# haoyuhsu/autovfx

Measured on AMD Instinct MI355X. Metric: rendered frames/sec at 1920x1080, 3M Gaussians, higher is better.
Workload: dtype f32; 1 GPU; C3: 3M synthetic Gaussians, 1920x1080, 800-frame orbit (BASELINE configs[2], per-GPU shard); P=3000000, sh_coeffs=16, width=1920, height=1080, tiles=8160, boundary=GaussianRasterizer.forward + RGBA8 pack per frame, parallelism=frame-parallel x1, streams_per_gpu=11, stream_driver=pipelined, n_ranks_seen=1

## Files before the change

autovfx_amd/csrc/gsr_binning.hip:

```cpp
#include "gsr_device.h"

#ifdef GSR_KERNEL_TRACE
__device__ unsigned long long* g_binning_trace = nullptr;
extern "C" __attribute__((visibility("default"))) int gsr_debug_set_binning_trace(void* device_words) {
    return (int)hipMemcpyToSymbol(HIP_SYMBOL(g_binning_trace), &device_words, sizeof device_words);
}
#define GSR_BTRACE(id, slot) do { if (threadIdx.x == 0 && g_binning_trace) g_binning_trace[(size_t)(id) * 8 + (slot)] = wall_clock64(); } while (0)
#else
#define GSR_BTRACE(id, slot) do { } while (0)
#endif

namespace gsr {
namespace {

constexpr int kPairTile = kExpandTile;
constexpr int kPairsPerLane = kPairTile / 256;
constexpr int kMaxDoneWords = 4096;
static_assert(kDupTile == 1024, "256 lanes x 4 consecutive positions");

__device__ __forceinline__ uint32_t block_sum_256(uint32_t v, uint32_t* scratch) {
#pragma unroll
    for (int d = 32; d >= 1; d >>= 1) v += (uint32_t)__shfl_xor((int)v, d);
    if ((threadIdx.x & 63) == 0) scratch[threadIdx.x >> 6] = v;
    __syncthreads();
    const uint32_t total = scratch[0] + scratch[1] + scratch[2] + scratch[3];
    __syncthreads();
    return total;
}

__device__ __forceinline__ uint32_t block_exclusive_256(uint32_t mine, uint32_t* s_wave, uint32_t* total) {
    const int lane = threadIdx.x & 63, wave = threadIdx.x >> 6;
    uint32_t incl = mine;
#pragma unroll
    for (int d = 1; d < 64; d <<= 1) {
        const uint32_t o = (uint32_t)__shfl_up((int)incl, d);
        if (lane >= d) incl += o;
    }
    if (lane == 63) s_wave[wave] = incl;
    __syncthreads();
    uint32_t before = incl - mine, all = 0;
#pragma unroll
    for (int w = 0; w < 4; ++w) {
        if (w < wave) before += s_wave[w];
        all += s_wave[w];
    }
    __syncthreads();
    *total = all;
    return before;
}

__device__ __forceinline__ bool rec_is_masked(uint32_t wh) { return (wh & 0xFFFFu) * (wh >> 16) <= kMaskTiles; }

__device__ __forceinline__ unsigned long long done_bits(const uint32_t* rows, int row_words, uint32_t ty, uint32_t x0, uint32_t w) {
    const uint32_t* r = rows + ty * (uint32_t)row_words;
    const uint32_t wi = x0 >> 5, sh = x0 & 31u;
    const uint32_t last = (uint32_t)row_words - 1u;
    const unsigned long long a = (unsigned long long)r[min(wi, last)] | ((unsigned long long)(wi + 1 <= last ? r[wi + 1] : 0u) << 32);
    unsigned long long v = a >> sh;
    if (sh + w > 64u) v |= (unsigned long long)(wi + 2 <= last ? r[wi + 2] : 0u) << (64u - sh);
    return w >= 64u ? v : v & ((1ull << w) - 1ull);
}

__device__ __forceinline__ unsigned long long done_rect(const uint32_t* rows, int row_words, uint32_t xy0, uint32_t wh) {
    const uint32_t x0 = xy0 & 0xFFFFu, y0 = xy0 >> 16, w = wh & 0xFFFFu, h = wh >> 16;
    unsigned long long d = 0ull;
    for (uint32_t j = 0; j < h; ++j) d |= done_bits(rows, row_words, y0 + j, x0, w) << (j * w);
    return d;
}

struct TileWalker {
    uint32_t x0, y0, width;
    bool masked;
    unsigned long long mask;
    float inv_width;
    const uint32_t* runs;
    const uint32_t* incl;
    const uint32_t* done;
    int row_words;
    uint32_t height, row, ca, cb, col_base, cur;

    __device__ __forceinline__ void load_run() {
        if (runs != nullptr) {
            const uint32_t r = runs[row];
            ca = r & 0xFFFFu; cb = r >> 16;
        } else {
            ca = x0; cb = x0 + width;
        }
    }
    __device__ __forceinline__ void load_word() {
        const uint32_t lo = max(ca, col_base), hi = min(cb, col_base + 32u);
// ... 84 lines not shown
    __shared__ float4 s_reg1[4][64];
    __shared__ uint4 s_geo[4][64];
    __shared__ uint32_t s_rows[4][64];
    __shared__ uint32_t s_live[4][64];
    const int tid = threadIdx.x, lane = tid & 63;
    const int V = a.V;
    const int k0 = (int)blockIdx.x * kDupTile + 4 * tid;
    GSR_BTRACE(blockIdx.x, 0);
    uint32_t gid[4] = {0u, 0u, 0u, 0u};
    if (k0 + 3 < V) {
        const uint4 g = *reinterpret_cast<const uint4*>(a.depth_order + k0);
        gid[0] = g.x; gid[1] = g.y; gid[2] = g.z; gid[3] = g.w;
    } else {
#pragma unroll
        for (int j = 0; j < 4; ++j)
            if (k0 + j < V) gid[j] = a.depth_order[k0 + j];
    }
    uint4 rec[4];
    uint32_t count[4];
    bool any_rows = false;
#pragma unroll
    for (int j = 0; j < 4; ++j) {
        rec[j] = make_uint4(0u, 0u, 0u, 0u);
        count[j] = 0u;
        if (k0 + j < V) {
            rec[j] = *reinterpret_cast<const uint4*>(a.bins + gid[j]);
            if (rec_is_masked(rec[j].y)) count[j] = (uint32_t)__popc(rec[j].z) + (uint32_t)__popc(rec[j].w);
            else if (a.tile_cull) {
                any_rows = true;
                rec[j].z += a.pool_first[gid[j] >> 8] + a.pool_group_first[gid[j] >> a.pool_group_shift];
            }
        }
    }
    const unsigned long long any_big = __ballot(any_rows);
    GSR_BTRACE(blockIdx.x, 1);
    if (any_big != 0ull) {
        const int wave = tid >> 6;
#pragma unroll
        for (int j = 0; j < 4; ++j) {
            const bool large = k0 + j < V && !rec_is_masked(rec[j].y);
            const uint32_t h = large ? rec[j].y >> 16 : 0u;
            const uint32_t pool_at = rec[j].z;
            bool walk = false;
            if (large) {
                if (pool_at > a.pool_rows || h > a.pool_rows - pool_at) {
                    rec[j].z = 0xFFFFFFFFu;
                    count[j] = (rec[j].y & 0xFFFFu) * h;
                    rec[j].w = count[j];
                } else {
                    walk = true;
                }
            }
            const uint32_t rows = walk ? h : 0u;
            uint32_t rincl = rows;
#pragma unroll
            for (int d = 1; d < 64; d <<= 1) {
                const uint32_t o = (uint32_t)__shfl_up((int)rincl, d);
                if (lane >= d) rincl += o;
            }
            const uint32_t total = (uint32_t)__shfl((int)rincl, 63);
            if (total != 0u) {
                if (walk) {
                    const float4* rr = reinterpret_cast<const float4*>(a.raster + gid[j]);
                    const float4 r0 = rr[0], r1 = rr[1];
                    const LiveRegion g = live_region(r0.z, r0.w, r1.x, r1.w);
                    s_reg0[wave][lane] = make_float4(g.A, g.B, g.C, g.beta);
                    s_reg1[wave][lane] = make_float4(g.u_ext, g.v_ext, r0.x, r0.y);
                    s_geo[wave][lane] = make_uint4(rec[j].x, (rec[j].y & 0xFFFFu) | ((uint32_t)g.kind << 16), pool_at, 0u);
                }
                s_rows[wave][lane] = rincl;
                s_live[wave][lane] = 0u;
                GSR_WAIT_LDS();
                __builtin_amdgcn_wave_barrier();
                for (uint32_t t0 = 0; t0 < total; t0 += 64u) {
                    const uint32_t t = t0 + (uint32_t)lane;
                    int lo = 64;
                    uint32_t len = 0u, before = 0u, pool_row = 0u, run = 0u;
                    if (t < total) {
                        lo = 0;
                        int hi = 63;
#pragma unroll
                        for (int step = 0; step < 6; ++step) {
                            const int mid = (lo + hi) >> 1;
                            if (s_rows[wave][mid] > t) hi = mid; else lo = mid + 1;
                        }
                        const uint32_t r = t - (lo > 0 ? s_rows[wave][lo - 1] : 0u);
                        const float4 q0 = s_reg0[wave][lo], q1 = s_reg1[wave][lo];
                        const uint4 ge = s_geo[wave][lo];
                        LiveRegion g;
                        g.A = q0.x; g.B = q0.y; g.C = q0.z; g.beta = q0.w; g.u_ext = q1.x; g.v_ext = q1.y; g.kind = (int)(ge.y >> 16);
                        const uint32_t x0 = ge.x & 0xFFFFu, y0 = ge.x >> 16, w = ge.y & 0xFFFFu;
                        int ca, cb;
                        row_run(g, q1.z, q1.w, (int)(y0 + r), (int)x0, (int)(x0 + w), &ca, &cb);
                        run = (uint32_t)ca | ((uint32_t)cb << 16);
                        len = (uint32_t)(cb - ca);
                        pool_row = ge.z + r;
                        before = s_live[wave][lo];
                    }
                    uint32_t incl_len = len;
#pragma unroll
                    for (int d = 1; d < 64; d <<= 1) {
                        const uint32_t o_len = (uint32_t)__shfl_up((int)incl_len, d);
                        const int o_seg = __shfl_up(lo, d);
                        if (lane >= d && o_seg == lo) incl_len += o_len;
                    }
                    GSR_WAIT_LDS();
                    __builtin_amdgcn_wave_barrier();
                    if (t < total) {
                        a.run_pool[pool_row] = run;
                        a.run_incl[pool_row] = before + incl_len;
                        if (len != 0u) atomicAdd(&s_live[wave][lo], len);
                    }
                    GSR_WAIT_LDS();
// ... 94 lines not shown
            slabs[0].pairs = mine[(below - 1u) & 3u];
            if (slabs_host != nullptr) slabs_host[0].pairs = mine[(below - 1u) & 3u];
        }
    }
}

__device__ __forceinline__ void load_done_rows(uint32_t* s_done, const uint32_t* __restrict__ done_rows, int words) {
    for (int i = threadIdx.x; i < words; i += 256) s_done[i] = done_rows[i];
    __syncthreads();
}

__global__ void __launch_bounds__(256, 7) slab_recount_kernel(BinningArrays a, int slab) {
    extern __shared__ uint32_t s_done[];
    __shared__ uint32_t s_wave[4];
    __shared__ uint4 s_geo[4][64];
    __shared__ uint32_t s_rows[4][64];
    __shared__ uint32_t s_live[4][64];
    GSR_BTRACE(8192 + blockIdx.x, 0);
    const SlabInfo info = a.slabs[slab];
    const uint32_t first = info.first, end = min(info.end, (uint32_t)a.V);
    const uint32_t k0 = first + blockIdx.x * (uint32_t)kDupTile + 4u * threadIdx.x;
    if (first + blockIdx.x * (uint32_t)kDupTile >= end) return;
    GSR_BTRACE(8192 + blockIdx.x, 1);
    load_done_rows(s_done, a.done_rows, a.grid_y * a.row_words);
    uint32_t done_tiles = 0;
    for (int i = threadIdx.x; i < a.grid_y * a.row_words; i += 256) {
        const int word = i % a.row_words;
        const uint32_t cols = (uint32_t)min(32, a.grid_x - 32 * word);
        done_tiles += (uint32_t)__popc(s_done[i] & (cols >= 32u ? ~0u : (1u << cols) - 1u));
    }
    const bool nothing_left = block_sum_256(done_tiles, s_wave) == (uint32_t)(a.grid_x * a.grid_y);
    GSR_BTRACE(8192 + blockIdx.x, 2);
    uint32_t count[4];
    uint4 rec[4];
#pragma unroll
    for (int j = 0; j < 4; ++j) {
        count[j] = 0u;
        rec[j] = make_uint4(0u, 0u, 0u, 0u);
        const uint32_t k = k0 + j;
        if (k >= end || nothing_left) continue;
        rec[j] = a.sorted_bins[k];
        if (rec[j].y == 0u || !rec_is_masked(rec[j].y)) continue;
        const unsigned long long m = (unsigned long long)rec[j].z | ((unsigned long long)rec[j].w << 32);
        const unsigned long long left = m & ~done_rect(s_done, a.row_words, rec[j].x, rec[j].y);
        count[j] = (uint32_t)__popcll(left);
    }
    GSR_BTRACE(8192 + blockIdx.x, 3);
    {
        const int lane = threadIdx.x & 63, wave = threadIdx.x >> 6;
#pragma unroll
        for (int j = 0; j < 4; ++j) {
            const bool large = k0 + j < end && rec[j].y != 0u && !rec_is_masked(rec[j].y);
            const uint32_t rows = large ? rec[j].y >> 16 : 0u;
            uint32_t rincl = rows;
#pragma unroll
            for (int d = 1; d < 64; d <<= 1) {
                const uint32_t o = (uint32_t)__shfl_up((int)rincl, d);
                if (lane >= d) rincl += o;
            }
            const uint32_t total = (uint32_t)__shfl((int)rincl, 63);
            if (total == 0u) continue;
            s_geo[wave][lane] = rec[j];
            s_rows[wave][lane] = rincl;
            s_live[wave][lane] = 0u;
            GSR_WAIT_LDS();
            __builtin_amdgcn_wave_barrier();
            for (uint32_t t0 = 0; t0 < total; t0 += 64u) {
                const uint32_t t = t0 + (uint32_t)lane;
                if (t < total) {
                    int lo = 0, hi = 63;
#pragma unroll
                    for (int step = 0; step < 6; ++step) {
                        const int mid = (lo + hi) >> 1;
                        if (s_rows[wave][mid] > t) hi = mid; else lo = mid + 1;
                    }
                    const uint32_t r = t - (lo > 0 ? s_rows[wave][lo - 1] : 0u);
                    const uint4 ge = s_geo[wave][lo];
                    const uint32_t x0 = ge.x & 0xFFFFu, y0 = ge.x >> 16, w = ge.y & 0xFFFFu;
                    uint32_t ca = x0, cb = x0 + w;
                    if (ge.z != 0xFFFFFFFFu) {
                        const uint32_t run = a.run_pool[ge.z + r];
                        ca = run & 0xFFFFu; cb = run >> 16;
                    }
                    uint32_t n = 0u;
                    for (uint32_t col = ca & ~31u; col < cb; col += 32u) {
                        const uint32_t lo_c = max(ca, col), hi_c = min(cb, col + 32u);
                        const uint32_t len = hi_c - lo_c;
                        uint32_t bits = (len >= 32u ? ~0u : ((1u << len) - 1u)) << (lo_c - col);
                        bits &= ~s_done[(y0 + r) * (uint32_t)a.row_words + (col >> 5)];
                        n += (uint32_t)__popc(bits);
                    }
                    if (n != 0u) atomicAdd(&s_live[wave][lo], n);
                }
            }
            GSR_WAIT_LDS();
            __builtin_amdgcn_wave_barrier();
            if (large) count[j] = s_live[wave][lane];
            __builtin_amdgcn_wave_barrier();
        }
    }
    GSR_BTRACE(8192 + blockIdx.x, 4);
    const uint32_t mine = count[0] + count[1] + count[2] + count[3];
    uint32_t tile_total;
    const uint32_t before = block_exclusive_256(mine, s_wave, &tile_total);
    const uint32_t emitting = (count[0] != 0u) + (count[1] != 0u) + (count[2] != 0u) + (count[3] != 0u);
    const uint32_t tile_emitting = block_sum_256(emitting, s_wave);
    if (threadIdx.x == 0) {
        a.slab_tile_totals[blockIdx.x] = tile_total;
        a.slab_tile_totals[a.tiles_p + blockIdx.x] = tile_emitting;
    }
    uint32_t run = before;
#pragma unroll
    for (int j = 0; j < 4; ++j) {
// ... 2 lines not shown
    }
    GSR_BTRACE(8192 + blockIdx.x, 5);
}

__global__ void __launch_bounds__(256) slab_compact_kernel(BinningArrays a, int slab) {
    __shared__ uint32_t s_scratch[4];
    __shared__ uint32_t s_wave[4];
    const SlabInfo info = a.slabs[slab];
    const uint32_t first = info.first, end = min(info.end, (uint32_t)a.V);
    const uint32_t tiles = end > first ? (end - first + kDupTile - 1) / kDupTile : 0u;
    const uint32_t* __restrict__ pair_totals = a.slab_tile_totals;
    const uint32_t* __restrict__ emit_totals = a.slab_tile_totals + a.tiles_p;
    if (blockIdx.x == 0) {
        uint32_t pp = 0, ee = 0;
        for (uint32_t t = threadIdx.x; t < tiles; t += 256) { pp += pair_totals[t]; ee += emit_totals[t]; }
        const uint32_t all_pairs = block_sum_256(pp, s_scratch);
        const uint32_t all_emit = block_sum_256(ee, s_scratch);
        if (threadIdx.x == 0) {
            a.slabs[slab].pairs = all_pairs; a.slabs[slab].emitters = all_emit;
            if (a.slabs_host != nullptr) a.slabs_host[slab].pairs = all_pairs;
        }
    }
    if (blockIdx.x >= tiles) return;
    uint32_t pp = 0, ee = 0;
    for (uint32_t t = threadIdx.x; t < blockIdx.x; t += 256) { pp += pair_totals[t]; ee += emit_totals[t]; }
    const uint32_t pairs_before = block_sum_256(pp, s_scratch);
    const uint32_t emit_before = block_sum_256(ee, s_scratch);
    const uint32_t tile_first = first + blockIdx.x * (uint32_t)kDupTile;
    const uint32_t k0 = tile_first + 4u * threadIdx.x;
    uint32_t incl[4], prev = 0u;
    if (threadIdx.x != 0 && k0 - 1u < end) prev = a.slab_offsets[k0 - 1u];
    uint32_t flags = 0u;
#pragma unroll
    for (int j = 0; j < 4; ++j) {
        incl[j] = k0 + j < end ? a.slab_offsets[k0 + j] : prev;
        if (incl[j] != prev) flags |= 1u << j;
        prev = incl[j];
    }
    uint32_t tile_emit;
    uint32_t rank = emit_before + block_exclusive_256((uint32_t)__popc(flags), s_wave, &tile_emit);
#pragma unroll
    for (int j = 0; j < 4; ++j) {
        if (k0 + j >= end) continue;
        const uint32_t global_incl = incl[j] + pairs_before;
        a.slab_offsets[k0 + j] = global_incl;
        if (flags & (1u << j)) {
            a.slab_cpos[rank] = k0 + j - first;
            a.slab_coffs[rank] = global_incl;
            ++rank;
        }
    }
}

__global__ void __launch_bounds__(256) expand_kernel(BinningArrays a, int slab, uint32_t* __restrict__ tile_keys,
                                                     uint32_t* __restrict__ point_list, uint32_t* __restrict__ first_counts,
                                                     uint32_t count_stride, uint32_t digit_mask) {
    constexpr int kBatch = 2048;
    __shared__ uint32_t s_incl[kBatch + 1];
    __shared__ uint32_t s_scratch[4];
    extern __shared__ uint32_t s_done[];
    const int tid = threadIdx.x;
    GSR_BTRACE(16384 + 8192 * slab + blockIdx.x, 0);
    const SlabInfo info = a.slabs[slab];
    const uint32_t num_pairs = info.pairs;
    const uint32_t per_lane = expand_pairs_per_lane(gridDim.x, num_pairs);
    const uint32_t pair_tile = 256u * per_lane;
    const uint32_t p_begin = blockIdx.x * pair_tile;
    if (p_begin >= num_pairs) return;
    const uint32_t p_end = min(num_pairs, p_begin + pair_tile);
    const uint32_t first = info.first;
    const bool compacted = slab > 0;
    const int V = compacted ? (int)info.emitters : (int)(min(info.end, (uint32_t)a.V) - first);
    const uint32_t* __restrict__ offsets = compacted ? a.slab_coffs : a.offsets + first;
    const uint32_t* __restrict__ cpos = a.slab_cpos;
    const uint4* __restrict__ sorted_bins = a.sorted_bins + first;
    const uint32_t* __restrict__ order = a.depth_order + first;
    const uint32_t* done = nullptr;
    if (slab > 0) {
        load_done_rows(s_done, a.done_rows, a.grid_y * a.row_words);
        done = s_done;
    }
    const uint32_t grid_x = (uint32_t)a.grid_x;
    GSR_BTRACE(16384 + 8192 * slab + blockIdx.x, 1);

    const int tiles = (V + kDupTile - 1) / kDupTile;
    uint32_t n_le = 0;
    for (int t = tid; t < tiles; t += 256) n_le += offsets[min((t + 1) * kDupTile, V) - 1] <= p_begin ? 1u : 0u;
    const int tile0 = (int)block_sum_256(n_le, s_scratch);
    n_le = 0;
    {
        const int k0 = tile0 * kDupTile + 4 * tid;
#pragma unroll
        for (int j = 0; j < 4; ++j)
            if (k0 + j < V) n_le += offsets[k0 + j] <= p_begin ? 1u : 0u;
    }
    int s0 = tile0 * kDupTile + (int)block_sum_256(n_le, s_scratch);
    auto position_of = [&](int item) -> uint32_t { return compacted ? cpos[item] : (uint32_t)item; };
    GSR_BTRACE(16384 + 8192 * slab + blockIdx.x, 2);

    const uint32_t my_begin = p_begin + per_lane * (uint32_t)tid;
    const uint32_t my_end = min(p_end, my_begin + per_lane);
    uint32_t keys[kPairsPerLane], ids[kPairsPerLane];
    while (s0 < V) {
        for (int i = tid; i <= kBatch; i += 256) {
            const int k = s0 - 1 + i;
            s_incl[i] = k < 0 ? 0u : offsets[min(k, V - 1)];
        }
        __syncthreads();
        const uint32_t lo_pair = max(my_begin, s_incl[0]);
        const uint32_t hi_pair = min(my_end, s_incl[kBatch]);
        if (lo_pair < hi_pair) {
            int lo = 1, hi = kBatch;
#pragma unroll
            for (int step = 0; step < 11; ++step) {
                const int mid = (lo + hi) >> 1;
                if (s_incl[mid] > lo_pair) hi = mid; else lo = mid + 1;
            }
            int owner = lo;
            uint32_t owner_end = s_incl[owner];
            TileWalker w;
            uint32_t pos = position_of(s0 + owner - 1);
            w.start(sorted_bins[pos], lo_pair - s_incl[owner - 1], a.run_pool, a.run_incl, done, a.row_words);
            uint32_t gid = order[pos];
            if (a.listed != nullptr) a.listed[gid] = (uint8_t)(slab + 1);
#pragma unroll
            for (int q = 0; q < kPairsPerLane; ++q) {
                const uint32_t p = my_begin + (uint32_t)q;
                if (p >= lo_pair && p < hi_pair) {
                    if (p >= owner_end) {
                        do { owner_end = s_incl[++owner]; } while (p >= owner_end);
                        pos = position_of(s0 + owner - 1);
                        w.start(sorted_bins[pos], 0u, a.run_pool, a.run_incl, done, a.row_words);
                        gid = order[pos];
                        if (a.listed != nullptr) a.listed[gid] = (uint8_t)(slab + 1);
                    }
                    keys[q] = w.next(grid_x);
                    ids[q] = gid;
                }
            }
        }
        const bool finished = s_incl[kBatch] >= p_end;
        __syncthreads();
        if (finished) break;
        s0 += kBatch;
    }
    GSR_BTRACE(16384 + 8192 * slab + blockIdx.x, 3);
    if (first_counts != nullptr) {
        uint32_t* s_hist = s_incl;
        __syncthreads();
        for (int i = tid; i < 4 * 256; i += 256) s_hist[i] = 0u;
        __syncthreads();
        uint32_t* mine = s_hist + 256 * (tid & 3);
#pragma unroll
        for (int q = 0; q < kPairsPerLane; ++q)
            if ((uint32_t)q < per_lane && my_begin + q < p_end) atomicAdd(&mine[keys[q] & digit_mask], 1u);
        __syncthreads();
        first_counts[(size_t)tid * count_stride + blockIdx.x] = s_hist[tid] + s_hist[256 + tid] + s_hist[512 + tid] + s_hist[768 + tid];
    }
    if (my_begin + per_lane <= p_end) {
#pragma unroll
        for (int q = 0; q < kPairsPerLane; q += 4) {
            if ((uint32_t)q >= per_lane) break;
            *reinterpret_cast<uint4*>(tile_keys + my_begin + q) = make_uint4(keys[q], keys[q + 1], keys[q + 2], keys[q + 3]);
            *reinterpret_cast<uint4*>(point_list + my_begin + q) = make_uint4(ids[q], ids[q + 1], ids[q + 2], ids[q + 3]);
        }
    } else {
#pragma unroll
        for (int q = 0; q < kPairsPerLane; ++q)
            if ((uint32_t)q < per_lane && my_begin + q < p_end) {
                tile_keys[my_begin + q] = keys[q];
                point_list[my_begin + q] = ids[q];
            }
    }
    GSR_BTRACE(16384 + 8192 * slab + blockIdx.x, 4);
}

__global__ void __launch_bounds__(256) tile_ranges_kernel(RangesDuty duty) {
    __shared__ uint32_t s_first[kRangesDutyLdsWords];
    tile_ranges_duty(duty, blockIdx.x, s_first);
}

__global__ void __launch_bounds__(256) list_order_check_kernel(const SlabInfo* __restrict__ slab, const uint32_t* __restrict__ keys,
                                                               const uint32_t* __restrict__ list,
                                                               const SplatRaster* __restrict__ raster, FrameCounters* counters) {
    const uint32_t n = slab->pairs;
    const uint32_t i = blockIdx.x * 256u + threadIdx.x + 1u;
    bool bad = false;
    if (i < n) {
        const uint32_t ta = keys[i - 1], tb = keys[i], ga = list[i - 1], gb = list[i];
        uint32_t da = __float_as_uint(raster[ga].depth), db = __float_as_uint(raster[gb].depth);
        if (da == kCulledKey) da = kCulledKey - 1u;
        if (db == kCulledKey) db = kCulledKey - 1u;
        bad = ta > tb || (ta == tb && (da > db || (da == db && ga >= gb)));
    }
    const unsigned long long b = __ballot(bad);
    if (b != 0ull && (threadIdx.x & 63) == 0) atomicAdd(&counters->order_violations, (uint32_t)__popcll(b));
}

}

hipError_t launch_list_order_check(const SlabInfo* slab, uint32_t pairs_bound, const uint32_t* sorted_tile_keys,
// ... 49 lines not shown
```

autovfx_amd/csrc/gsr_device.h:

```cpp
#pragma once
#include "gsr_internal.h"

namespace gsr {
namespace {

inline int div_up(int a, int b) { return (a + b - 1) / b; }

#define GSR_WAIT_LDS() __builtin_amdgcn_s_waitcnt(0xC07F)

__device__ __forceinline__ uint32_t lower_bound_u32(const uint32_t* __restrict__ a, uint32_t n, uint32_t v) {
    uint32_t lo = 0, hi = n;
    while (lo < hi) {
        const uint32_t mid = lo + ((hi - lo) >> 1);
        if (a[mid] < v) lo = mid + 1; else hi = mid;
    }
    return lo;
}

constexpr int kRangesDutyLdsWords = 256 + 2 * 8 * kOrderClasses;

__device__ __forceinline__ void tile_ranges_duty(const RangesDuty& d, uint32_t block, uint32_t* s_first ) {
    if (block == 0 && threadIdx.x < 3 && d.header_dst[threadIdx.x] != nullptr)
        *reinterpret_cast<ArenaHeader*>(d.header_dst[threadIdx.x]) = d.headers[threadIdx.x];
    const int t = (int)block * 255 + (int)threadIdx.x;
    const uint32_t n = d.slab->pairs;
    uint32_t* s_cell = s_first + 256;
    const bool ordering = d.order.counts != nullptr;
    if (ordering && threadIdx.x < 2 * 8 * kOrderClasses) s_cell[threadIdx.x] = 0u;
    s_first[threadIdx.x] = lower_bound_u32(d.keys, n, (uint32_t)min(t, d.num_tiles));
    __syncthreads();
    const bool mine = threadIdx.x != 255 && t < d.num_tiles;
    int cell = 0;
    uint32_t rank = 0u;
    if (mine) {
        const uint32_t b = s_first[threadIdx.x], e = s_first[threadIdx.x + 1];
        d.ranges[t] = (e > b) ? make_uint2(b, e) : make_uint2(0u, 0u);
        if (ordering) {
            const int xcd = (t / d.order.strip) & 7;
            const uint32_t len = e > b ? e - b : 0u;
            const int cls = len == 0u ? kOrderClasses - 1 : (kOrderClasses - 2) - (int)min((uint32_t)(kOrderClasses - 2), len >> d.order.shift);
            cell = xcd * kOrderClasses + cls;
            rank = atomicAdd(&s_cell[cell], 1u);
        }
    }
    if (ordering) {
        __syncthreads();
        if (threadIdx.x < 8 * kOrderClasses && s_cell[threadIdx.x] != 0u)
            s_cell[8 * kOrderClasses + threadIdx.x] = atomicAdd(&d.order.counts[threadIdx.x], s_cell[threadIdx.x]);
        __syncthreads();
        if (mine) d.order.table[(size_t)cell * d.order.cap + s_cell[8 * kOrderClasses + cell] + rank] = (uint32_t)t;
    }
    __syncthreads();
}

struct __attribute__((aligned(4))) F3 { float x, y, z; };
struct __attribute__((aligned(4))) F4 { float x, y, z, w; };

struct Mat3 { float m[3][3]; };

__device__ __forceinline__ Mat3 mul3(const Mat3& a, const Mat3& b) {
    Mat3 r;
#pragma unroll
    for (int i = 0; i < 3; ++i)
#pragma unroll
        for (int j = 0; j < 3; ++j)
            r.m[i][j] = a.m[i][0] * b.m[0][j] + a.m[i][1] * b.m[1][j] + a.m[i][2] * b.m[2][j];
    return r;
}
__device__ __forceinline__ Mat3 transpose3(const Mat3& a) {
    Mat3 r;
#pragma unroll
    for (int i = 0; i < 3; ++i)
#pragma unroll
        for (int j = 0; j < 3; ++j) r.m[i][j] = a.m[j][i];
    return r;
}

__device__ __forceinline__ int f2i_sat(float v) {
    if (v != v) return 0;
    if (v >= 2147483648.0f) return 2147483647;
    if (v <= -2147483648.0f) return (-2147483647 - 1);
    return (int)v;
}

__device__ __forceinline__ float ndc_to_pix(float v, int S) {
    return (float)((((double)v + 1.0) * (double)S - 1.0) * 0.5);
}

struct TileRect { int x0, y0, x1, y1; };

__device__ __forceinline__ TileRect tile_rect(float px, float py, int radius, int gx, int gy) {
    TileRect r;
    r.x0 = min(gx, max(0, f2i_sat((px - radius) / kTile)));
    r.y0 = min(gy, max(0, f2i_sat((py - radius) / kTile)));
    r.x1 = min(gx, max(0, f2i_sat((px + radius + kTile - 1) / kTile)));
    r.y1 = min(gy, max(0, f2i_sat((py + radius + kTile - 1) / kTile)));
    return r;
}

constexpr float kSH0 = 0.28209479177387814f;
constexpr float kSH1 = 0.4886025119029199f;
constexpr float kSH2_0 = 1.0925484305920792f, kSH2_1 = -1.0925484305920792f, kSH2_2 = 0.31539156525252005f,
                kSH2_3 = -1.0925484305920792f, kSH2_4 = 0.5462742152960396f;
constexpr float kSH3_0 = -0.5900435899266435f, kSH3_1 = 2.890611442640554f, kSH3_2 = -0.4570457994644658f,
                kSH3_3 = 0.3731763325901154f, kSH3_4 = -0.4570457994644658f, kSH3_5 = 1.445305721320277f,
// ... 228 lines not shown
```

autovfx_amd/csrc/gsr_kernels.hip:

```cpp
#include "gsr_device.h"

#include <cstring>

#ifdef GSR_KERNEL_TRACE
__device__ unsigned long long* g_kernel_trace = nullptr;
extern "C" __attribute__((visibility("default"))) int gsr_debug_set_trace(void* device_words) {
    return (int)hipMemcpyToSymbol(HIP_SYMBOL(g_kernel_trace), &device_words, sizeof device_words);
}
#define GSR_KTRACE(id, slot) do { if (threadIdx.x == 0 && g_kernel_trace) g_kernel_trace[(size_t)(id) * 8 + (slot)] = wall_clock64(); } while (0)
#else
#define GSR_KTRACE(id, slot) do { } while (0)
#endif

namespace gsr {
namespace {

template <bool kRaw>
__global__ void __launch_bounds__(256) preprocess_kernel(GaussianInputs in, Camera cam, GeometryArrays out) {
    const int i = blockIdx.x * 256 + threadIdx.x;
    const bool in_range = i < in.P;
    GSR_KTRACE(blockIdx.x, 0);

    const float* __restrict__ vm = cam.viewmatrix;
    const float* __restrict__ pm = cam.projmatrix;

    int radius_out = 0;
    uint32_t rect_area = 0;
    uint32_t live_bound = 0;
    uint32_t big_rows = 0;
    bool violation = false;
    SplatBin bin = {0u, 0u, 0u, 0u};
    uint32_t key = kCulledKey;
    bool mask_candidate = false;
    uint32_t cand_rows = 0;
    LiveRegion cand_region = {0.f, 0.f, 0.f, 0.f, 0.f, 0.f, 0};
    float2 cand_centre = make_float2(0.f, 0.f);

    if (in_range) {
    if (out.ids != nullptr) out.ids[i] = (uint32_t)i;
    const F3 p = ld3(in.means3D + 3 * (size_t)i);

    const float hx = pm[0] * p.x + pm[4] * p.y + pm[8] * p.z + pm[12];
    const float hy = pm[1] * p.x + pm[5] * p.y + pm[9] * p.z + pm[13];
    const float hw = pm[3] * p.x + pm[7] * p.y + pm[11] * p.z + pm[15];
    const float vx = vm[0] * p.x + vm[4] * p.y + vm[8] * p.z + vm[12];
    const float vy = vm[1] * p.x + vm[5] * p.y + vm[9] * p.z + vm[13];
    const float vz = vm[2] * p.x + vm[6] * p.y + vm[10] * p.z + vm[14];

    if (vz <= 0.2f) {
        violation = in.prefiltered != 0;
    } else {
        const float pw = 1.0f / (hw + 0.0000001f);
        const float ndc_x = hx * pw, ndc_y = hy * pw;

        float c3[6];
        F3 s = {0.f, 0.f, 0.f};
        F4 q = {0.f, 0.f, 0.f, 0.f};
        if (in.cov3D_precomp != nullptr) {
            const float* c = in.cov3D_precomp + 6 * (size_t)i;
#pragma unroll
            for (int k = 0; k < 6; ++k) c3[k] = c[k];
        } else {
            s = ld3(in.scales + 3 * (size_t)i);
            q = *reinterpret_cast<const F4*>(in.rotations + 4 * (size_t)i);
            if (kRaw) {
                s = F3{expf(s.x), expf(s.y), expf(s.z)};
                q = torch_normalize4(q);
            }
            const float r = q.x, x = q.y, y = q.z, z = q.w;
            Mat3 S = {{{in.scale_modifier * s.x, 0.f, 0.f}, {0.f, in.scale_modifier * s.y, 0.f},
                       {0.f, 0.f, in.scale_modifier * s.z}}};
            Mat3 R;
            R.m[0][0] = 1.f - 2.f * (y * y + z * z); R.m[1][0] = 2.f * (x * y - r * z);       R.m[2][0] = 2.f * (x * z + r * y);
            R.m[0][1] = 2.f * (x * y + r * z);       R.m[1][1] = 1.f - 2.f * (x * x + z * z); R.m[2][1] = 2.f * (y * z - r * x);
            R.m[0][2] = 2.f * (x * z - r * y);       R.m[1][2] = 2.f * (y * z + r * x);       R.m[2][2] = 1.f - 2.f * (x * x + y * y);
            const Mat3 Mm = mul3(S, R);
            const Mat3 Sg = mul3(transpose3(Mm), Mm);
            c3[0] = Sg.m[0][0]; c3[1] = Sg.m[1][0]; c3[2] = Sg.m[2][0];
            c3[3] = Sg.m[1][1]; c3[4] = Sg.m[2][1]; c3[5] = Sg.m[2][2];
        }

        const float limx = 1.3f * cam.tan_fovx, limy = 1.3f * cam.tan_fovy;
        const float txtz = vx / vz, tytz = vy / vz;
        const float tx = fminf(limx, fmaxf(-limx, txtz)) * vz;
        const float ty = fminf(limy, fmaxf(-limy, tytz)) * vz;
        Mat3 J = {{{cam.focal_x / vz, 0.f, 0.f}, {0.f, cam.focal_y / vz, 0.f},
                   {-(cam.focal_x * tx) / (vz * vz), -(cam.focal_y * ty) / (vz * vz), 0.f}}};
        Mat3 Wm;
#pragma unroll
        for (int a = 0; a < 3; ++a)
#pragma unroll
            for (int b = 0; b < 3; ++b) Wm.m[a][b] = vm[4 * a + b];
        const Mat3 T = mul3(Wm, J);
        Mat3 V = {{{c3[0], c3[1], c3[2]}, {c3[1], c3[3], c3[4]}, {c3[2], c3[4], c3[5]}}};
        const Mat3 cov = mul3(mul3(transpose3(T), transpose3(V)), T);
        const float ca = cov.m[0][0] + 0.3f, cb = cov.m[1][0], cc = cov.m[1][1] + 0.3f;

        const float det = ca * cc - cb * cb;
        if (det != 0.0f) {
            const float det_inv = 1.f / det;
            const float mid = 0.5f * (ca + cc);
            const float lam1 = mid + sqrtf(fmaxf(0.1f, mid * mid - det));
            const float lam2 = mid - sqrtf(fmaxf(0.1f, mid * mid - det));
            const float rad = ceilf(3.f * sqrtf(fmaxf(lam1, lam2)));
            const float px = ndc_to_pix(ndc_x, cam.width), py = ndc_to_pix(ndc_y, cam.height);
            const int irad = f2i_sat(rad);
            const TileRect rc = tile_rect(px, py, irad, cam.grid_x, cam.grid_y);
            const uint32_t area = (uint32_t)(rc.x1 - rc.x0) * (uint32_t)(rc.y1 - rc.y0);
            if (area != 0) {
                if (in.colors_precomp == nullptr && !in.defer_colour) {
                    int deg = in.sh_degree < 3 ? in.sh_degree : 3;
                    if (deg > 2 && in.M < 16) deg = 2;
                    if (deg > 1 && in.M < 9) deg = 1;
                    if (deg > 0 && in.M < 4) deg = 0;
                    const F3 cp = ld3(cam.cam_pos);
                    const float* sh0 = kRaw ? in.shs + 3 * (size_t)i : in.shs + 3 * (size_t)in.M * i;
                    const float* shr = (kRaw && in.M > 1) ? in.shs_rest + 3 * (size_t)(in.M - 1) * i - 3 : sh0;
                    const F3 col = sh_to_rgb(deg, p, cp, sh0, shr);
                    *reinterpret_cast<F3*>(out.rgb + 3 * (size_t)i) = col;
                }
                if (kRaw && in.view_normals != nullptr)
                    *reinterpret_cast<F3*>(in.view_normals + 3 * (size_t)i) = view_normal_rgb(p, ld3(cam.cam_pos), min_axis(s, q));
                const float opacity = kRaw ? torch_sigmoid(in.opacities[i]) : in.opacities[i];
                const float4 conic_o = make_float4(cc * det_inv, -cb * det_inv, ca * det_inv, opacity);
                float4* rec = reinterpret_cast<float4*>(out.raster + i);
                rec[0] = make_float4(px, py, conic_o.x, conic_o.y);
                const float skip_below = blend_skip_below(conic_o.w);
                rec[1] = make_float4(conic_o.z, conic_o.w, vz, skip_below);
                radius_out = irad;
                rect_area = area;
                TileRect tr = rc;
                LiveRegion region = {0.f, 0.f, 0.f, 0.f, 0.f, 0.f, 0};
                if (in.tile_cull) {
                    region = live_region(conic_o.x, conic_o.y, conic_o.z, skip_below);
                    tr = tight_rect(region, px, py, rc);
                }
                const uint32_t tw = (uint32_t)(tr.x1 - tr.x0), th = (uint32_t)(tr.y1 - tr.y0), tarea = tw * th;
                if (tarea != 0u && irad > 0) {
                    bin.xy0 = (uint32_t)tr.x0 | ((uint32_t)tr.y0 << 16);
                    bin.wh = tw | (th << 16);
                    if (tarea <= kMaskTiles) {
                        const unsigned long long all = tarea == 64u ? ~0ull : (1ull << tarea) - 1ull;
                        bin.lo = (uint32_t)all; bin.hi = (uint32_t)(all >> 32);
                        live_bound = tarea;
                        if (in.tile_cull && tw >= 2u && th >= 2u && region.kind == 1) {
                            mask_candidate = true;
                            cand_rows = th;
                            cand_region = region;
                            cand_centre = make_float2(px, py);
                        }
                    } else {
                        bin.lo = bin.hi = 0xFFFFFFFFu;
                        live_bound = tarea;
                        big_rows = th;
                    }
                    key = __float_as_uint(vz);
                    if (key == kCulledKey) key = kCulledKey - 1u;
                }
            }
        }
    }
    }
    GSR_KTRACE(blockIdx.x, 1);

    {
        __shared__ float4 s_reg0[4][64];
        __shared__ float4 s_reg1[4][64];
        __shared__ uint2 s_place[4][64];
        __shared__ uint32_t s_incl[4][64];
        __shared__ uint32_t s_mask[4][64][2];
        const int lane = threadIdx.x & 63, wave = threadIdx.x >> 6;
        uint32_t incl = cand_rows;
#pragma unroll
        for (int d = 1; d < 64; d <<= 1) {
            const uint32_t o = (uint32_t)__shfl_up((int)incl, d);
            if (lane >= d) incl += o;
        }
        const uint32_t total = (uint32_t)__shfl((int)incl, 63);
        if (total != 0u) {
            s_reg0[wave][lane] = make_float4(cand_region.A, cand_region.B, cand_region.C, cand_region.beta);
            s_reg1[wave][lane] = make_float4(cand_region.u_ext, cand_region.v_ext, cand_centre.x, cand_centre.y);
            s_place[wave][lane] = make_uint2(bin.xy0, bin.wh & 0xFFFFu);
            s_incl[wave][lane] = incl;
            s_mask[wave][lane][0] = 0u;
            s_mask[wave][lane][1] = 0u;
            GSR_WAIT_LDS();
            __builtin_amdgcn_wave_barrier();
            for (uint32_t t0 = 0; t0 < total; t0 += 64u) {
                const uint32_t t = t0 + (uint32_t)lane;
                if (t < total) {
                    int lo = 0, hi = 63;
#pragma unroll
                    for (int step = 0; step < 6; ++step) {
                        const int mid = (lo + hi) >> 1;
                        if (s_incl[wave][mid] > t) hi = mid; else lo = mid + 1;
                    }
                    const uint32_t r = t - (lo > 0 ? s_incl[wave][lo - 1] : 0u);
                    const float4 q0 = s_reg0[wave][lo], q1 = s_reg1[wave][lo];
                    const uint2 pl = s_place[wave][lo];
                    LiveRegion g;
                    g.A = q0.x; g.B = q0.y; g.C = q0.z; g.beta = q0.w; g.u_ext = q1.x; g.v_ext = q1.y; g.kind = 1;
                    const uint32_t x0 = pl.x & 0xFFFFu, y0 = pl.x >> 16, w = pl.y;
                    int ca, cb;
                    row_run<true>(g, q1.z, q1.w, (int)(y0 + r), (int)x0, (int)(x0 + w), &ca, &cb);
                    if (cb > ca) {
                        const uint32_t len = (uint32_t)(cb - ca);
                        const unsigned long long bits = ((len >= 32u ? 0xFFFFFFFFull : (1ull << len) - 1ull) << ((uint32_t)ca - x0)) << (r * w);
                        if ((uint32_t)bits != 0u) atomicOr(&s_mask[wave][lo][0], (uint32_t)bits);
                        if ((uint32_t)(bits >> 32) != 0u) atomicOr(&s_mask[wave][lo][1], (uint32_t)(bits >> 32));
                    }
                }
            }
            GSR_WAIT_LDS();
            __builtin_amdgcn_wave_barrier();
            if (mask_candidate) {
                const unsigned long long mask = ((unsigned long long)s_mask[wave][lane][0] | ((unsigned long long)s_mask[wave][lane][1] << 32)) &
                                                ((unsigned long long)bin.lo | ((unsigned long long)bin.hi << 32));
                bin.lo = (uint32_t)mask; bin.hi = (uint32_t)(mask >> 32);
                live_bound = (uint32_t)__popcll(mask);
                if (mask == 0ull) {
                    bin.wh = 0u;
                    key = kCulledKey;
                }
            }
        }
    }

    GSR_KTRACE(blockIdx.x, 2);
    __shared__ unsigned long long s_tot[4];
    __shared__ uint32_t s_vis[4], s_big[4];
    unsigned long long wave_tot = ((unsigned long long)rect_area << 32) | (unsigned long long)live_bound;
#pragma unroll
    for (int d = 32; d >= 1; d >>= 1) wave_tot += __shfl_xor(wave_tot, d);
    const unsigned long long emitting = __ballot(key != kCulledKey);
    const unsigned long long any_big = __ballot(big_rows != 0u);
    uint32_t big_incl = big_rows;
    if (any_big != 0ull) {
#pragma unroll
        for (int d = 1; d < 64; d <<= 1) {
            const uint32_t o = (uint32_t)__shfl_up((int)big_incl, d);
            if ((int)(threadIdx.x & 63) >= d) big_incl += o;
        }
    }
    const unsigned long long any_violation = __ballot(violation);
    if ((threadIdx.x & 63) == 63) {
        const int w = threadIdx.x >> 6;
        s_tot[w] = wave_tot;
        s_vis[w] = (uint32_t)__popcll(emitting);
        s_big[w] = big_incl | (any_violation != 0ull ? 0x80000000u : 0u);
    }
    __syncthreads();
    if (big_rows != 0u) {
        uint32_t before = big_incl - big_rows;
        for (int w = 0; w < (int)(threadIdx.x >> 6); ++w) before += s_big[w] & 0x7FFFFFFFu;
        bin.lo = before;
    }
    if (in_range) {
        out.radii[i] = radius_out;
        *reinterpret_cast<uint4*>(out.bins + i) = make_uint4(bin.xy0, bin.wh, bin.lo, bin.hi);
        out.depth_keys[i] = key;
        if (out.listed != nullptr) out.listed[i] = 0u;
    }
    if (threadIdx.x == 0) {
        BlockTally t;
        t.pair_total = s_tot[0] + s_tot[1] + s_tot[2] + s_tot[3];
        t.visible = s_vis[0] + s_vis[1] + s_vis[2] + s_vis[3];
        const uint32_t big = (s_big[0] & 0x7FFFFFFFu) + (s_big[1] & 0x7FFFFFFFu) + (s_big[2] & 0x7FFFFFFFu) + (s_big[3] & 0x7FFFFFFFu);
        t.big_rows = big | ((s_big[0] | s_big[1] | s_big[2] | s_big[3]) & 0x80000000u);
        *reinterpret_cast<uint4*>(out.tallies + blockIdx.x) = *reinterpret_cast<const uint4*>(&t);
    }
    GSR_KTRACE(blockIdx.x, 3);
}

__global__ void __launch_bounds__(256) sh_colour_listed_kernel(GaussianInputs in, const float* __restrict__ cam_pos,
                                                               const uint8_t* __restrict__ listed, int tag,
                                                               const SlabInfo* __restrict__ slab, float* __restrict__ rgb,
                                                               RangesDuty duty, int duty_blocks) {
    __shared__ uint32_t s_list[4][256];
    GSR_KTRACE(16384 + 8192 * (tag - 1) + blockIdx.x, 0);
    if ((int)blockIdx.x < duty_blocks) tile_ranges_duty(duty, blockIdx.x, &s_list[0][0]);
    GSR_KTRACE(16384 + 8192 * (tag - 1) + blockIdx.x, 1);
    const int lane = threadIdx.x & 63, wave = threadIdx.x >> 6;
    const int first = (blockIdx.x * 4 + wave) * 256;
    if (first >= in.P || slab->pairs == 0u) return;
    const int i0 = first + 4 * lane;
    uint32_t marks = 0u;
    if (i0 + 3 < in.P) marks = *reinterpret_cast<const uint32_t*>(listed + i0);
    else
        for (int j = 0; j < 4; ++j)
            if (i0 + j < in.P) marks |= (uint32_t)listed[i0 + j] << (8 * j);
    bool mine[4];
    uint32_t cnt = 0u;
#pragma unroll
    for (int j = 0; j < 4; ++j) {
        mine[j] = ((marks >> (8 * j)) & 0xFFu) == (uint32_t)tag;
        cnt += mine[j] ? 1u : 0u;
    }
    uint32_t incl = cnt;
#pragma unroll
    for (int d = 1; d < 64; d <<= 1) {
        const uint32_t o = (uint32_t)__shfl_up((int)incl, d);
        if (lane >= d) incl += o;
    }
    const uint32_t n = (uint32_t)__shfl((int)incl, 63);
    uint32_t at = incl - cnt;
#pragma unroll
    for (int j = 0; j < 4; ++j)
        if (mine[j]) s_list[wave][at++] = (uint32_t)(i0 + j);
    GSR_KTRACE(16384 + 8192 * (tag - 1) + blockIdx.x, 2);
    if (n == 0u) return;
    __builtin_amdgcn_s_waitcnt(0);
    __builtin_amdgcn_wave_barrier();
    int deg = in.sh_degree < 3 ? in.sh_degree : 3;
    if (deg > 2 && in.M < 16) deg = 2;
    if (deg > 1 && in.M < 9) deg = 1;
    if (deg > 0 && in.M < 4) deg = 0;
    const F3 cp = ld3(cam_pos);
    for (uint32_t t = (uint32_t)lane; t < n; t += 64u) {
        const uint32_t i = s_list[wave][t];
        const F3 p = ld3(in.means3D + 3 * (size_t)i);
        const float* sh0 = in.raw ? in.shs + 3 * (size_t)i : in.shs + 3 * (size_t)in.M * i;
        const float* shr = (in.raw && in.M > 1) ? in.shs_rest + 3 * (size_t)(in.M - 1) * i - 3 : sh0;
        const F3 col = sh_to_rgb(deg, p, cp, sh0, shr);
        *reinterpret_cast<F3*>(rgb + 3 * (size_t)i) = col;
    }
    GSR_KTRACE(16384 + 8192 * (tag - 1) + blockIdx.x, 3);
}

__global__ void __launch_bounds__(256) sh_colour_all_kernel(GaussianInputs in, const float* __restrict__ cam_pos,
                                                            const int* __restrict__ radii, float* __restrict__ rgb,
                                                            RangesDuty duty, int duty_blocks) {
    __shared__ uint32_t s_first[kRangesDutyLdsWords];
    if ((int)blockIdx.x < duty_blocks) tile_ranges_duty(duty, blockIdx.x, s_first);
    const int i = blockIdx.x * 256 + threadIdx.x;
    if (i >= in.P || radii[i] <= 0) return;
    int deg = in.sh_degree < 3 ? in.sh_degree : 3;
    if (deg > 2 && in.M < 16) deg = 2;
    if (deg > 1 && in.M < 9) deg = 1;
    if (deg > 0 && in.M < 4) deg = 0;
    const F3 p = ld3(in.means3D + 3 * (size_t)i);
    const float* sh0 = in.raw ? in.shs + 3 * (size_t)i : in.shs + 3 * (size_t)in.M * i;
    const float* shr = (in.raw && in.M > 1) ? in.shs_rest + 3 * (size_t)(in.M - 1) * i - 3 : sh0;
    const F3 col = sh_to_rgb(deg, p, ld3(cam_pos), sh0, shr);
    *reinterpret_cast<F3*>(rgb + 3 * (size_t)i) = col;
}

__global__ void __launch_bounds__(256) mark_visible_kernel(int P, const float* __restrict__ means3D,
                                                           const float* __restrict__ vm,
                                                           uint8_t* __restrict__ present) {
    const int i = blockIdx.x * 256 + threadIdx.x;
    if (i >= P) return;
    const F3 p = ld3(means3D + 3 * (size_t)i);
    const float vz = vm[2] * p.x + vm[6] * p.y + vm[10] * p.z + vm[14];
    present[i] = (uint8_t)(vz > 0.2f);
}

__device__ __forceinline__ uint32_t quantize8(float v) {
// ... 419 lines not shown
```

Baseline: 1514 frames/s.

## Use DPP wave scans, stage expand records in LDS, slim preprocess state

Replaces the shuffle-based wave prefix sums and reductions across binning and preprocess kernels with a DPP-based inclusive scan plus readlane. The expand kernel now processes smaller chunks and stages the sorted bin records and gids in shared memory, so lanes no longer issue scattered global loads on owner changes. It also uses precomputed tile totals for the starting search and sets a launch-bounds occupancy hint. The preprocess kernel drops several per-thread temporaries in favour of writing candidate regions straight to LDS, aiming to lower register pressure. The DPP row-broadcast scan pattern and the larger shared footprint in expand could affect correctness or occupancy.

```diff
diff --git a/autovfx_amd/csrc/gsr_binning.hip b/autovfx_amd/csrc/gsr_binning.hip
--- a/autovfx_amd/csrc/gsr_binning.hip
+++ b/autovfx_amd/csrc/gsr_binning.hip
@@ -19,8 +19,7 @@
 static_assert(kDupTile == 1024, "256 lanes x 4 consecutive positions");
 
 __device__ __forceinline__ uint32_t block_sum_256(uint32_t v, uint32_t* scratch) {
-#pragma unroll
-    for (int d = 32; d >= 1; d >>= 1) v += (uint32_t)__shfl_xor((int)v, d);
+    v = wave_sum(v);
     if ((threadIdx.x & 63) == 0) scratch[threadIdx.x >> 6] = v;
     __syncthreads();
     const uint32_t total = scratch[0] + scratch[1] + scratch[2] + scratch[3];
@@ -30,12 +29,7 @@
 
 __device__ __forceinline__ uint32_t block_exclusive_256(uint32_t mine, uint32_t* s_wave, uint32_t* total) {
     const int lane = threadIdx.x & 63, wave = threadIdx.x >> 6;
-    uint32_t incl = mine;
-#pragma unroll
-    for (int d = 1; d < 64; d <<= 1) {
-        const uint32_t o = (uint32_t)__shfl_up((int)incl, d);
-        if (lane >= d) incl += o;
-    }
+    const uint32_t incl = wave_inclusive_scan(mine);
     if (lane == 63) s_wave[wave] = incl;
     __syncthreads();
     uint32_t before = incl - mine, all = 0;
@@ -226,13 +220,8 @@
                 }
             }
             const uint32_t rows = walk ? h : 0u;
-            uint32_t rincl = rows;
-#pragma unroll
-            for (int d = 1; d < 64; d <<= 1) {
-                const uint32_t o = (uint32_t)__shfl_up((int)rincl, d);
-                if (lane >= d) rincl += o;
-            }
-            const uint32_t total = (uint32_t)__shfl((int)rincl, 63);
+            const uint32_t rincl = wave_inclusive_scan(rows);
+            const uint32_t total = (uint32_t)__builtin_amdgcn_readlane((int)rincl, 63);
             if (total != 0u) {
                 if (walk) {
                     const float4* rr = reinterpret_cast<const float4*>(a.raster + gid[j]);
@@ -433,13 +422,8 @@
         for (int j = 0; j < 4; ++j) {
             const bool large = k0 + j < end && rec[j].y != 0u && !rec_is_masked(rec[j].y);
             const uint32_t rows = large ? rec[j].y >> 16 : 0u;
-            uint32_t rincl = rows;
-#pragma unroll
-            for (int d = 1; d < 64; d <<= 1) {
-                const uint32_t o = (uint32_t)__shfl_up((int)rincl, d);
-                if (lane >= d) rincl += o;
-            }
-            const uint32_t total = (uint32_t)__shfl((int)rincl, 63);
+            const uint32_t rincl = wave_inclusive_scan(rows);
+            const uint32_t total = (uint32_t)__builtin_amdgcn_readlane((int)rincl, 63);
             if (total == 0u) continue;
             s_geo[wave][lane] = rec[j];
             s_rows[wave][lane] = rincl;
@@ -548,11 +532,14 @@
     }
 }
 
-__global__ void __launch_bounds__(256) expand_kernel(BinningArrays a, int slab, uint32_t* __restrict__ tile_keys,
+__global__ void __launch_bounds__(256, 7) expand_kernel(BinningArrays a, int slab, uint32_t* __restrict__ tile_keys,
                                                      uint32_t* __restrict__ point_list, uint32_t* __restrict__ first_counts,
                                                      uint32_t count_stride, uint32_t digit_mask) {
-    constexpr int kBatch = 2048;
-    __shared__ uint32_t s_incl[kBatch + 1];
+    constexpr int kChunk = 768;
+    constexpr int kChunkLoads = kChunk / 256;
+    __shared__ uint32_t s_incl[kChunk + 1];
+    __shared__ uint4 s_rec[kChunk];
+    __shared__ uint32_t s_gid[kChunk];
     __shared__ uint32_t s_scratch[4];
     extern __shared__ uint32_t s_done[];
     const int tid = threadIdx.x;
@@ -581,7 +568,11 @@
 
     const int tiles = (V + kDupTile - 1) / kDupTile;
     uint32_t n_le = 0;
-    for (int t = tid; t < tiles; t += 256) n_le += offsets[min((t + 1) * kDupTile, V) - 1] <= p_begin ? 1u : 0u;
+    const uint32_t* __restrict__ tile_ends = (!compacted && first == 0u) ? a.tile_totals + a.tiles_p : nullptr;
+    for (int t = tid; t < tiles; t += 256) {
+        const uint32_t tile_end = (tile_ends != nullptr && (t + 1) * kDupTile <= V) ? tile_ends[t] : offsets[min((t + 1) * kDupTile, V) - 1];
+        n_le += tile_end <= p_begin ? 1u : 0u;
+    }
     const int tile0 = (int)block_sum_256(n_le, s_scratch);
     n_le = 0;
     {
@@ -591,43 +582,56 @@
             if (k0 + j < V) n_le += offsets[k0 + j] <= p_begin ? 1u : 0u;
     }
     int s0 = tile0 * kDupTile + (int)block_sum_256(n_le, s_scratch);
-    auto position_of = [&](int item) -> uint32_t { return compacted ? cpos[item] : (uint32_t)item; };
     GSR_BTRACE(16384 + 8192 * slab + blockIdx.x, 2);
 
     const uint32_t my_begin = p_begin + per_lane * (uint32_t)tid;
     const uint32_t my_end = min(p_end, my_begin + per_lane);
     uint32_t keys[kPairsPerLane], ids[kPairsPerLane];
     while (s0 < V) {
-        for (int i = tid; i <= kBatch; i += 256) {
-            const int k = s0 - 1 + i;
-            s_incl[i] = k < 0 ? 0u : offsets[min(k, V - 1)];
+        uint32_t before[kChunkLoads], pos[kChunkLoads];
+#pragma unroll
+        for (int j = 0; j < kChunkLoads; ++j) {
+            const int i = tid + 256 * j, k = s0 - 1 + i;
+            before[j] = k < 0 ? 0u : offsets[min(k, V - 1)];
+            pos[j] = (uint32_t)(s0 + i);
+            if (compacted && s0 + i < V) pos[j] = cpos[s0 + i];
+        }
+        if (tid == 0) s_incl[kChunk] = offsets[min(s0 - 1 + kChunk, V - 1)];
+#pragma unroll
+        for (int j = 0; j < kChunkLoads; ++j) {
+            const int i = tid + 256 * j;
+            s_incl[i] = before[j];
+            if (s0 + i < V && before[j] < p_end) {
+                s_rec[i] = sorted_bins[pos[j]];
+                s_gid[i] = order[pos[j]];
+            }
         }
         __syncthreads();
         const uint32_t lo_pair = max(my_begin, s_incl[0]);
-        const uint32_t hi_pair = min(my_end, s_incl[kBatch]);
+        const uint32_t hi_pair = min(my_end, s_incl[kChunk]);
         if (lo_pair < hi_pair) {
-            int lo = 1, hi = kBatch;
-#pragma unroll
-            for (int step = 0; step < 11; ++step) {
+            int lo = 1, hi = kChunk;
+#pragma unroll
+            for (int step = 0; step < 10; ++step) {
                 const int mid = (lo + hi) >> 1;
                 if (s_incl[mid] > lo_pair) hi = mid; else lo = mid + 1;
             }
             int owner = lo;
             uint32_t owner_end = s_incl[owner];
             TileWalker w;
-            uint32_t pos = position_of(s0 + owner - 1);
-            w.start(sorted_bins[pos], lo_pair - s_incl[owner - 1], a.run_pool, a.run_incl, done, a.row_words);
-            uint32_t gid = order[pos];
+            w.start(s_rec[owner - 1], lo_pair - s_incl[owner - 1], a.run_pool, a.run_incl, done, a.row_words);
+            uint32_t gid = s_gid[owner - 1];
             if (a.listed != nullptr) a.listed[gid] = (uint8_t)(slab + 1);
+            uint32_t p0 = my_begin;
+            asm("" : "+v"(p0));
 #pragma unroll
             for (int q = 0; q < kPairsPerLane; ++q) {
-                const uint32_t p = my_begin + (uint32_t)q;
+                const uint32_t p = p0 + (uint32_t)q;
                 if (p >= lo_pair && p < hi_pair) {
                     if (p >= owner_end) {
                         do { owner_end = s_incl[++owner]; } while (p >= owner_end);
-                        pos = position_of(s0 + owner - 1);
-                        w.start(sorted_bins[pos], 0u, a.run_pool, a.run_incl, done, a.row_words);
-                        gid = order[pos];
+                        w.start(s_rec[owner - 1], 0u, a.run_pool, a.run_incl, done, a.row_words);
+                        gid = s_gid[owner - 1];
                         if (a.listed != nullptr) a.listed[gid] = (uint8_t)(slab + 1);
                     }
                     keys[q] = w.next(grid_x);
@@ -635,14 +639,14 @@
                 }
             }
         }
-        const bool finished = s_incl[kBatch] >= p_end;
+        const bool finished = s_incl[kChunk] >= p_end;
         __syncthreads();
         if (finished) break;
-        s0 += kBatch;
+        s0 += kChunk;
     }
     GSR_BTRACE(16384 + 8192 * slab + blockIdx.x, 3);
     if (first_counts != nullptr) {
-        uint32_t* s_hist = s_incl;
+        uint32_t* s_hist = reinterpret_cast<uint32_t*>(s_rec);
         __syncthreads();
         for (int i = tid; i < 4 * 256; i += 256) s_hist[i] = 0u;
         __syncthreads();
diff --git a/autovfx_amd/csrc/gsr_device.h b/autovfx_amd/csrc/gsr_device.h
--- a/autovfx_amd/csrc/gsr_device.h
+++ b/autovfx_amd/csrc/gsr_device.h
@@ -51,6 +51,31 @@
         if (mine) d.order.table[(size_t)cell * d.order.cap + s_cell[8 * kOrderClasses + cell] + rank] = (uint32_t)t;
     }
     __syncthreads();
+}
+
+constexpr int kDppRowShr = 0x110, kDppRowBcast15 = 0x142, kDppRowBcast31 = 0x143;
+
+struct WaveDpp {
+    template <int kCtrl, int kRowMask>
+    static __device__ __forceinline__ uint32_t moved(uint32_t v) {
+        return (uint32_t)__builtin_amdgcn_update_dpp(0, (int)v, kCtrl, kRowMask, 0xF, false);
+    }
+};
+
+template <class Moves, class T>
+__host__ __device__ __forceinline__ T wave_scan_steps(T v) {
+    v = v + Moves::template moved<kDppRowShr + 1, 0xF>(v);
+    v = v + Moves::template moved<kDppRowShr + 2, 0xF>(v);
+    v = v + Moves::template moved<kDppRowShr + 4, 0xF>(v);
+    v = v + Moves::template moved<kDppRowShr + 8, 0xF>(v);
+    v = v + Moves::template moved<kDppRowBcast15, 0xA>(v);
+    v = v + Moves::template moved<kDppRowBcast31, 0xC>(v);
+    return v;
+}
+
+__device__ __forceinline__ uint32_t wave_inclusive_scan(uint32_t v) { return wave_scan_steps<WaveDpp>(v); }
+__device__ __forceinline__ uint32_t wave_sum(uint32_t v) {
+    return (uint32_t)__builtin_amdgcn_readlane((int)wave_inclusive_scan(v), 63);
 }
 
 struct __attribute__((aligned(4))) F3 { float x, y, z; };
diff --git a/autovfx_amd/csrc/gsr_kernels.hip b/autovfx_amd/csrc/gsr_kernels.hip
--- a/autovfx_amd/csrc/gsr_kernels.hip
+++ b/autovfx_amd/csrc/gsr_kernels.hip
@@ -26,15 +26,17 @@
 
     int radius_out = 0;
     uint32_t rect_area = 0;
-    uint32_t live_bound = 0;
-    uint32_t big_rows = 0;
     bool violation = false;
-    SplatBin bin = {0u, 0u, 0u, 0u};
+    uint32_t bin_xy0 = 0u, bin_wh = 0u;
     uint32_t key = kCulledKey;
-    bool mask_candidate = false;
     uint32_t cand_rows = 0;
-    LiveRegion cand_region = {0.f, 0.f, 0.f, 0.f, 0.f, 0.f, 0};
-    float2 cand_centre = make_float2(0.f, 0.f);
+    asm("" : "+v"(radius_out), "+v"(rect_area), "+v"(bin_xy0), "+v"(bin_wh), "+v"(key), "+v"(cand_rows));
+    __shared__ float4 s_reg0[4][64];
+    __shared__ float4 s_reg1[4][64];
+    __shared__ uint2 s_place[4][64];
+    __shared__ uint32_t s_incl[4][64];
+    __shared__ uint32_t s_mask[4][64][2];
+    const int lane = threadIdx.x & 63, wave = threadIdx.x >> 6;
 
     if (in_range) {
     if (out.ids != nullptr) out.ids[i] = (uint32_t)i;
@@ -137,22 +139,13 @@
                 }
                 const uint32_t tw = (uint32_t)(tr.x1 - tr.x0), th = (uint32_t)(tr.y1 - tr.y0), tarea = tw * th;
                 if (tarea != 0u && irad > 0) {
-                    bin.xy0 = (uint32_t)tr.x0 | ((uint32_t)tr.y0 << 16);
-                    bin.wh = tw | (th << 16);
-                    if (tarea <= kMaskTiles) {
-                        const unsigned long long all = tarea == 64u ? ~0ull : (1ull << tarea) - 1ull;
-                        bin.lo = (uint32_t)all; bin.hi = (uint32_t)(all >> 32);
-                        live_bound = tarea;
-                        if (in.tile_cull && tw >= 2u && th >= 2u && region.kind == 1) {
-                            mask_candidate = true;
-                            cand_rows = th;
-                            cand_region = region;
-                            cand_centre = make_float2(px, py);
-                        }
-                    } else {
-                        bin.lo = bin.hi = 0xFFFFFFFFu;
-                        live_bound = tarea;
-                        big_rows = th;
+                    bin_xy0 = (uint32_t)tr.x0 | ((uint32_t)tr.y0 << 16);
+                    bin_wh = tw | (th << 16);
+                    if (in.tile_cull && tarea <= kMaskTiles && tw >= 2u && th >= 2u && region.kind == 1) {
+                        cand_rows = th;
+                        s_reg0[wave][lane] = make_float4(region.A, region.B, region.C, region.beta);
+                        s_reg1[wave][lane] = make_float4(region.u_ext, region.v_ext, px, py);
+                        s_place[wave][lane] = make_uint2(bin_xy0, tw);
                     }
                     key = __float_as_uint(vz);
                     if (key == kCulledKey) key = kCulledKey - 1u;
@@ -163,24 +156,15 @@
     }
     GSR_KTRACE(blockIdx.x, 1);
 
+    const uint32_t tiles = (bin_wh & 0xFFFFu) * (bin_wh >> 16);
+    const bool big = tiles > (uint32_t)kMaskTiles;
+    const uint32_t big_rows = big ? bin_wh >> 16 : 0u;
+    unsigned long long payload = big ? ~0ull : tiles == 64u ? ~0ull : (1ull << tiles) - 1ull;
+    uint32_t live_bound = tiles;
     {
-        __shared__ float4 s_reg0[4][64];
-        __shared__ float4 s_reg1[4][64];
-        __shared__ uint2 s_place[4][64];
-        __shared__ uint32_t s_incl[4][64];
-        __shared__ uint32_t s_mask[4][64][2];
-        const int lane = threadIdx.x & 63, wave = threadIdx.x >> 6;
-        uint32_t incl = cand_rows;
-#pragma unroll
-        for (int d = 1; d < 64; d <<= 1) {
-            const uint32_t o = (uint32_t)__shfl_up((int)incl, d);
-            if (lane >= d) incl += o;
-        }
-        const uint32_t total = (uint32_t)__shfl((int)incl, 63);
+        const uint32_t incl = wave_inclusive_scan(cand_rows);
+        const uint32_t total = (uint32_t)__builtin_amdgcn_readlane((int)incl, 63);
         if (total != 0u) {
-            s_reg0[wave][lane] = make_float4(cand_region.A, cand_region.B, cand_region.C, cand_region.beta);
-            s_reg1[wave][lane] = make_float4(cand_region.u_ext, cand_region.v_ext, cand_centre.x, cand_centre.y);
-            s_place[wave][lane] = make_uint2(bin.xy0, bin.wh & 0xFFFFu);
             s_incl[wave][lane] = incl;
             s_mask[wave][lane][0] = 0u;
             s_mask[wave][lane][1] = 0u;
@@ -213,13 +197,11 @@
             }
             GSR_WAIT_LDS();
             __builtin_amdgcn_wave_barrier();
-            if (mask_candidate) {
-                const unsigned long long mask = ((unsigned long long)s_mask[wave][lane][0] | ((unsigned long long)s_mask[wave][lane][1] << 32)) &
-                                                ((unsigned long long)bin.lo | ((unsigned long long)bin.hi << 32));
-                bin.lo = (uint32_t)mask; bin.hi = (uint32_t)(mask >> 32);
-                live_bound = (uint32_t)__popcll(mask);
-                if (mask == 0ull) {
-                    bin.wh = 0u;
+            if (cand_rows != 0u) {
+                payload &= (unsigned long long)s_mask[wave][lane][0] | ((unsigned long long)s_mask[wave][lane][1] << 32);
+                live_bound = (uint32_t)__popcll(payload);
+                if (payload == 0ull) {
+                    bin_wh = 0u;
                     key = kCulledKey;
                 }
             }
@@ -229,35 +211,24 @@
     GSR_KTRACE(blockIdx.x, 2);
     __shared__ unsigned long long s_tot[4];
     __shared__ uint32_t s_vis[4], s_big[4];
-    unsigned long long wave_tot = ((unsigned long long)rect_area << 32) | (unsigned long long)live_bound;
-#pragma unroll
-    for (int d = 32; d >= 1; d >>= 1) wave_tot += __shfl_xor(wave_tot, d);
+    const unsigned long long wave_tot = ((unsigned long long)wave_sum(rect_area) << 32) | (unsigned long long)wave_sum(live_bound);
     const unsigned long long emitting = __ballot(key != kCulledKey);
-    const unsigned long long any_big = __ballot(big_rows != 0u);
-    uint32_t big_incl = big_rows;
-    if (any_big != 0ull) {
-#pragma unroll
-        for (int d = 1; d < 64; d <<= 1) {
-            const uint32_t o = (uint32_t)__shfl_up((int)big_incl, d);
-            if ((int)(threadIdx.x & 63) >= d) big_incl += o;
-        }
-    }
+    const uint32_t big_incl = wave_inclusive_scan(big_rows);
     const unsigned long long any_violation = __ballot(violation);
-    if ((threadIdx.x & 63) == 63) {
-        const int w = threadIdx.x >> 6;
-        s_tot[w] = wave_tot;
-        s_vis[w] = (uint32_t)__popcll(emitting);
-        s_big[w] = big_incl | (any_violation != 0ull ? 0x80000000u : 0u);
+    if (lane == 63) {
+        s_tot[wave] = wave_tot;
+        s_vis[wave] = (uint32_t)__popcll(emitting);
+        s_big[wave] = big_incl | (any_violation != 0ull ? 0x80000000u : 0u);
     }
     __syncthreads();
     if (big_rows != 0u) {
         uint32_t before = big_incl - big_rows;
-        for (int w = 0; w < (int)(threadIdx.x >> 6); ++w) before += s_big[w] & 0x7FFFFFFFu;
-        bin.lo = before;
+        for (int w = 0; w < wave; ++w) before += s_big[w] & 0x7FFFFFFFu;
+        payload = 0xFFFFFFFF00000000ull | before;
     }
     if (in_range) {
         out.radii[i] = radius_out;
-        *reinterpret_cast<uint4*>(out.bins + i) = make_uint4(bin.xy0, bin.wh, bin.lo, bin.hi);
+        *reinterpret_cast<uint4*>(out.bins + i) = make_uint4(bin_xy0, bin_wh, (uint32_t)payload, (uint32_t)(payload >> 32));
         out.depth_keys[i] = key;
         if (out.listed != nullptr) out.listed[i] = 0u;
     }
@@ -296,13 +267,8 @@
         mine[j] = ((marks >> (8 * j)) & 0xFFu) == (uint32_t)tag;
         cnt += mine[j] ? 1u : 0u;
     }
-    uint32_t incl = cnt;
-#pragma unroll
-    for (int d = 1; d < 64; d <<= 1) {
-        const uint32_t o = (uint32_t)__shfl_up((int)incl, d);
-        if (lane >= d) incl += o;
-    }
-    const uint32_t n = (uint32_t)__shfl((int)incl, 63);
+    const uint32_t incl = wave_inclusive_scan(cnt);
+    const uint32_t n = (uint32_t)__builtin_amdgcn_readlane((int)incl, 63);
     uint32_t at = incl - cnt;
 #pragma unroll
     for (int j = 0; j < 4; ++j)
```

Result: faster. 1551 frames/s, median of 6 (+2.4%).
